# tgp-team/torch-geometric-pool

Hardware: AMD Instinct MI355X
Metric: pooled nodes/sec (Reduce+Connect) on batched graphs (higher is better)
Workload: dtype f32; 1 GPU; DiffPool dense S^T X / S^T A S, batch=32 graphs N=1024 K=128 F=64 (BASELINE configs[1]); graphs_per_gpu=32, nodes_per_graph=1024, clusters=128, features=64, parallelism=graph-sharded x1

## Files before the change

torch-geometric-pool_amd/csrc/dense.hip:

```cpp
#include <stdlib.h>

#include "common.h"
#include "gemm_mfma.h"
#include "dense_post.h"
#include "dense_graph_kernels.h"

namespace tgp {

static const int kStage2Tile = getenv("TGP_STAGE2_TILE") ? atoi(getenv("TGP_STAGE2_TILE")) : 0;
static const int kStage2TileM = getenv("TGP_STAGE2_TILE_M") ? atoi(getenv("TGP_STAGE2_TILE_M")) : 0;
struct DensePlan {
  int splits, tile, tile_m;
  int k_per_split;
  size_t u_floats, aslab_floats, xslab_floats, post_floats, colsum_floats;
};

static DensePlan dense_plan(int64_t B, int64_t N, int64_t K, int64_t F, bool with_gram = false) {
  DensePlan p;
  p.tile = (kStage2Tile == 64 || kStage2Tile == 128) ? kStage2Tile : 64;
  p.tile_m = (kStage2TileM == 64 || kStage2TileM == 128) ? kStage2TileM : p.tile;
  const int64_t T = p.tile, TM = p.tile_m;
  const int64_t tiles = ((K + TM - 1) / TM) * ((with_gram ? 2 : 1) * ((K + T - 1) / T) + ((F + T - 1) / T));
  const int64_t base = B * (tiles > 0 ? tiles : 1);
  const int64_t max_splits = (N + 4 * BK - 1) / (4 * BK);
  const int64_t cus = 256;
  int64_t splits = 1;
  double best = 1e30;
  for (int64_t sp = 1; sp <= 32 && sp <= (max_splits > 0 ? max_splits : 1); ++sp) {
    const int64_t wgs = base * sp;
    const int64_t ksteps = ((N + sp - 1) / sp + BK - 1) / BK;
    const int64_t per_cu = (wgs + cus - 1) / cus, resident = per_cu < 4 ? per_cu : 4;
    const double cost = static_cast<double>((per_cu + 3) / 4) * static_cast<double>(ksteps + 3) *
                        static_cast<double>(2 + resident) * (1.0 + 0.01 * sp);
    if (cost < best) { best = cost; splits = sp; }
  }
  static const int force_splits = getenv("TGP_STAGE2_SPLITS") ? atoi(getenv("TGP_STAGE2_SPLITS")) : 0;
  if (force_splits > 0 && force_splits <= max_splits) splits = force_splits;
  int64_t kps = (N + splits - 1) / splits;
  kps = (kps + BK - 1) / BK * BK;
  splits = (N + kps - 1) / kps;
  if (splits < 1) splits = 1;
  p.splits = static_cast<int>(splits);
  p.k_per_split = static_cast<int>(kps);
  p.u_floats = static_cast<size_t>(B) * N * K;
  const int64_t fold = fold_tiles(N, K, F) <= PR_MAX_SPLITS ? fold_tiles(N, K, F) : 0;
  const int64_t slabs = splits > fold ? splits : fold;
  const int64_t parts = splits * ((K + 63) / 64) > fold ? splits * ((K + 63) / 64) : fold;
  p.aslab_floats = static_cast<size_t>(B) * slabs * K * K;
  p.xslab_floats = static_cast<size_t>(B) * slabs * K * F;
  p.post_floats = post_ws_floats(B, K);
  p.colsum_floats = static_cast<size_t>(B) * parts * K;
  return p;
}

}

using namespace tgp;

extern "C" size_t tgp_dense_pool_workspace_bytes(int64_t B, int64_t N, int64_t K, int64_t F) {
  if (B <= 0 || N <= 0 || K <= 0) return 256;
  const DensePlan p = dense_plan(B, N, K, F > 0 ? F : 0);
  return align_up(p.u_floats * 4) + align_up(p.aslab_floats * 4) + align_up(p.xslab_floats * 4) +
         align_up(p.post_floats * 4) + align_up(p.colsum_floats * 4) + 256;
}

static bool dense_pool_small_ok(int64_t B, int64_t N, int64_t K, int64_t F) {
  static const int no_small = getenv("TGP_NO_SMALL_GRAPH_KERNEL") ? 1 : 0;
  return !no_small && N <= SG_N && K <= SG_K && F <= SG_K && B >= 64;
}

extern "C" int tgp_dense_pool_is_small(int64_t B, int64_t N, int64_t K, int64_t F) {
  return dense_pool_small_ok(B, N, K, F) ? 1 : 0;
}

static int dense_pool_impl(const float* S, const float* A, const float* X, int64_t B, int64_t N, int64_t K, int64_t F,
                           int flags, float eps, const int64_t* graph_sizes, float* x_pool, float* adj_raw,
                           float* adj_pool, float* mincut_terms, float loss_eps, void* ws, size_t ws_bytes,
                           void* stream_);
static int dense_pool_tiled(const float* S, const float* A, const float* X, int64_t B, int64_t N, int64_t K, int64_t F,
                            int flags, float eps, float* x_pool, float* adj_raw, float* adj_pool, float* U, int64_t ldu,
                            float* gram, const DensePlan& p, Carver& cv, hipStream_t stream, bool keep_u = true);

extern "C" int tgp_dense_pool_f32(const float* S, const float* A, const float* X, int64_t B, int64_t N,
                                  int64_t K, int64_t F, int flags, float eps, const int64_t* graph_sizes,
                                  float* x_pool,
                                  float* adj_raw, float* adj_pool, void* ws, size_t ws_bytes, void* stream_) {
  return dense_pool_impl(S, A, X, B, N, K, F, flags, eps, graph_sizes, x_pool, adj_raw, adj_pool, nullptr, 0.f, ws,
                         ws_bytes, stream_);
}

extern "C" int tgp_dense_pool_mincut_f32(const float* S, const float* A, const float* X, int64_t B, int64_t N,
                                         int64_t K, int64_t F, int flags, float eps, float loss_eps, float* x_pool,
                                         float* adj_raw, float* adj_pool, float* mincut_terms, void* ws,
                                         size_t ws_bytes, void* stream_) {
  TGP_REQUIRE(mincut_terms && A, TGP_ERR_INVALID, "tgp_dense_pool_mincut_f32: mincut_terms / A is null");
  TGP_REQUIRE(dense_pool_small_ok(B, N, K, F), TGP_ERR_INVALID,
              "tgp_dense_pool_mincut_f32: only batches the one-wave-per-graph kernel takes (tgp_dense_pool_is_small)");
  return dense_pool_impl(S, A, X, B, N, K, F, flags, eps, nullptr, x_pool, adj_raw, adj_pool, mincut_terms, loss_eps,
                         ws, ws_bytes, stream_);
}

extern "C" int tgp_dense_pool_select_f32(const float* X, const float* A, const float* W, const float* bias,
                                         const unsigned char* mask, int64_t B, int64_t N, int64_t K, int64_t F,
                                         int flags, float eps, float loss_eps, float* S_out, float* x_pool,
// ... 140 lines not shown
    (void)hipFuncSetAttribute(reinterpret_cast<const void*>(dense_pool_small_kernel<false, true>),
                              hipFuncAttributeMaxDynamicSharedMemorySize,
                              static_cast<int>(SG_WAVES * SG_WAVE_FLOATS * sizeof(float)));
    hipLaunchKernelGGL((dense_pool_small_kernel<false, true>), dim3(grid), dim3(64 * SG_WAVES),
                       SG_WAVES * SG_WAVE_FLOATS * sizeof(float), stream, q);
    return check_launch("tgp_dense_pool_f32(small)");
  }
  static const int no_medium = getenv("TGP_NO_MEDIUM_GRAPH_KERNEL") ? 1 : 0;
  static const int kMediumMinGraphs = getenv("TGP_MEDIUM_MIN_GRAPHS") ? atoi(getenv("TGP_MEDIUM_MIN_GRAPHS")) : 8;
  static const int kMediumMaxLds = getenv("TGP_MEDIUM_MAX_LDS") ? atoi(getenv("TGP_MEDIUM_MAX_LDS")) : 152 * 1024;
  if (!no_medium && K <= 64 && B >= kMediumMinGraphs && reinterpret_cast<uintptr_t>(S) % 4 == 0) {
    const int64_t npad = (N + 31) / 32 * 32;
    const size_t lds = K <= 32 ? medium_lds_bytes<1>(npad) : medium_lds_bytes<2>(npad);
    const bool fits32 = static_cast<int64_t>(N) * (N > F ? N : F) * 4 < (1ll << 31) - 4096;
    if (lds <= static_cast<size_t>(kMediumMaxLds) && fits32) {
      MediumArgs q{S, want_a ? A : nullptr, want_x ? X : nullptr, static_cast<int>(B), static_cast<int>(N),
                   static_cast<int>(K), static_cast<int>(F), flags, eps, want_x ? x_pool : nullptr,
                   want_a ? adj_raw : nullptr, want_a ? adj_pool : nullptr, static_cast<int>(npad), graph_sizes};
      static const int force_waves = getenv("TGP_MEDIUM_WAVES") ? atoi(getenv("TGP_MEDIUM_WAVES")) : 0;
      const int64_t strips = (want_a ? (N + 31) / 32 : 0) + (want_x ? (F + 31) / 32 : 0);
      const bool eight = force_waves ? force_waves == 8 : (strips >= 8 && lds > 80 * 1024);
      const dim3 g(static_cast<unsigned>(B));
      if (K <= 32) {
        if (eight) hipLaunchKernelGGL((dense_pool_medium_kernel<1, 4, 8>), g, dim3(512), lds, stream, q);
        else hipLaunchKernelGGL((dense_pool_medium_kernel<1>), g, dim3(256), lds, stream, q);
      } else {
        if (eight) hipLaunchKernelGGL((dense_pool_medium_kernel<2, 2, 8>), g, dim3(512), lds, stream, q);
        else hipLaunchKernelGGL((dense_pool_medium_kernel<2, 2>), g, dim3(256), lds, stream, q);
      }
      return check_launch("tgp_dense_pool_f32(medium)");
    }
  }
  TGP_REQUIRE(ws && ws_bytes >= tgp_dense_pool_workspace_bytes(B, N, K, F), TGP_ERR_WORKSPACE,
              "tgp_dense_pool_f32: workspace too small");
  const DensePlan p = dense_plan(B, N, K, F);
  Carver cv(ws);
  float* U = cv.take<float>(p.u_floats);
  return dense_pool_tiled(S, A, X, B, N, K, F, flags, eps, x_pool, adj_raw, adj_pool, U, K, nullptr, p, cv, stream,
                          false);
}

static int dense_pool_tiled(const float* S, const float* A, const float* X, int64_t B, int64_t N, int64_t K, int64_t F,
                            int flags, float eps, float* x_pool, float* adj_raw, float* adj_pool, float* U, int64_t ldu,
                            float* gram, const DensePlan& p, Carver& cv, hipStream_t stream, bool keep_u) {
  const bool want_x = X && x_pool && F > 0;
  const bool want_a = A && (adj_raw || adj_pool);
  float* aslab = cv.take<float>(p.aslab_floats);
  float* xslab = cv.take<float>(p.xslab_floats);
  float* postws = cv.take<float>(p.post_floats);
  float* colpart = cv.take<float>(p.colsum_floats);
  float* gslab = gram ? cv.take<float>(p.aslab_floats) : nullptr;

  const int fold = (want_a && !keep_u && !gram) ? fold_tiles(N, K, F) : 0;
  if (fold > 0 && fold <= PR_MAX_SPLITS && static_cast<size_t>(B) * fold * K * K <= p.aslab_floats &&
      post_rows_ok(K, flags, aslab, adj_raw, adj_pool) &&
      reinterpret_cast<uintptr_t>(xslab) % 16 == 0) {
    GemmArgs g{};
    g.A = A; g.lda = N; g.sA = N * N;
    g.M = static_cast<int>(N); g.Kd = static_cast<int>(N);
    g.rhs[0] = GemmRhs{S, aslab, static_cast<int>(K), K, K, N * K, static_cast<long>(fold) * K * K, K * K};
    if (want_x) g.rhs[1] = GemmRhs{X, xslab, static_cast<int>(F), F, F, N * F, static_cast<long>(fold) * K * F, K * F};
    g.splits = 1; g.k_per_split = static_cast<int>((N + BK - 1) / BK * BK);
    g.colsum = colpart;
    g.colsum_skip_diag = (flags & TGP_REMOVE_SELF_LOOPS) ? 1 : 0;
    const bool folded = (flags & TGP_ADJ_TRANSPOSED) ? launch_gemm_fold<true>(g, static_cast<int>(B), stream)
                                                     : launch_gemm_fold<false>(g, static_cast<int>(B), stream);
    if (folded) {
      PostRowsArgs r{};
      r.slab = aslab; r.splits = fold; r.s_split = K * K; r.s_batch = static_cast<long>(fold) * K * K;
      r.colsum = (flags & TGP_DEGREE_NORM) ? colpart : nullptr; r.tiles_m = 1;
      r.K = static_cast<int>(K); r.flags = flags; r.eps = eps; r.raw = adj_raw; r.dst = adj_pool;
      if (want_x) {
        r.xslab = xslab; r.xs_split = K * F; r.xs_batch = static_cast<long>(fold) * K * F;
        r.F = static_cast<int>(F); r.x_pool = x_pool;
      }
      const unsigned grid = static_cast<unsigned>(B * ((K + PR_ROWS - 1) / PR_ROWS));
      r.main_blocks = static_cast<int>(grid);
      hipLaunchKernelGGL(post_rows_kernel, dim3(grid), dim3(512), 0, stream, r);
      return check_launch("tgp_dense_pool_f32");
    }
  }
  if (want_a) {
    GemmArgs g{};
    g.A = A; g.lda = N; g.sA = N * N;
    g.M = static_cast<int>(N); g.Kd = static_cast<int>(N);
    g.rhs[0] = GemmRhs{S, U, static_cast<int>(K), K, ldu, N * K, N * ldu, 0};
    g.splits = 1; g.k_per_split = static_cast<int>((N + BK - 1) / BK * BK);
    if (flags & TGP_ADJ_TRANSPOSED) launch_gemm_skip_zeros<true>(g, static_cast<int>(B), stream);
    else launch_gemm_skip_zeros<false>(g, static_cast<int>(B), stream);
  }
  if (want_a || want_x) {
    GemmArgs h{};
    h.A = S; h.lda = K; h.sA = N * K;
    h.M = static_cast<int>(K); h.Kd = static_cast<int>(N);
    h.splits = p.splits; h.k_per_split = p.k_per_split;
    h.force_bm = p.tile_m; h.force_bn = p.tile;
    const GemmRhs ra{U, aslab, static_cast<int>(K), ldu, K, N * ldu, static_cast<long>(p.splits) * K * K, K * K};
    const GemmRhs rx{X, xslab, static_cast<int>(F), F, F, N * F, static_cast<long>(p.splits) * K * F, K * F};
    const GemmRhs rg{S, gslab, static_cast<int>(K), K, K, N * K, static_cast<long>(p.splits) * K * K, K * K};
    int nr = 0;
    if (want_a) h.rhs[nr++] = ra;
    if (want_x) h.rhs[nr++] = rx;
    if (gram) h.rhs[nr++] = rg;
    if (want_a && post_rows_ok(K, flags, aslab, adj_raw, adj_pool) && p.tile == 64 && p.tile_m == 64 &&
        p.splits <= PR_MAX_SPLITS && p.splits * ((K + 63) / 64) <= 2 * PR_MAX_SPLITS) {
      h.colsum = colpart;
      h.colsum_skip_diag = (flags & TGP_REMOVE_SELF_LOOPS) ? 1 : 0;
    }
    int tiles_m = 0;
    const bool have_colsum = launch_gemm<true>(h, static_cast<int>(B), stream, &tiles_m);
    if (have_colsum) {
      PostRowsArgs r{};
      r.slab = aslab; r.splits = p.splits; r.s_split = K * K; r.s_batch = static_cast<long>(p.splits) * K * K;
      r.colsum = (flags & TGP_DEGREE_NORM) ? colpart : nullptr; r.tiles_m = tiles_m;
      r.K = static_cast<int>(K); r.flags = flags; r.eps = eps; r.raw = adj_raw; r.dst = adj_pool;
      if (want_x) {
        r.xslab = xslab; r.xs_split = K * F; r.xs_batch = static_cast<long>(p.splits) * K * F;
        r.F = static_cast<int>(F); r.x_pool = x_pool;
      }
      unsigned grid = static_cast<unsigned>(B * ((K + PR_ROWS - 1) / PR_ROWS));
      r.main_blocks = static_cast<int>(grid);
      if (gram) {
        r.gslab = gslab; r.gram = gram;
        grid *= 2;
      }
      hipLaunchKernelGGL(post_rows_kernel, dim3(grid), dim3(512), 0, stream, r);
      return check_launch("tgp_dense_pool_f32");
    }
  }
  if (gram) {
    const long total = K * K;
    int gx = static_cast<int>((total + 255) / 256);
    if (gx > 64) gx = 64;
    hipLaunchKernelGGL(combine_slabs_kernel, dim3(gx, static_cast<unsigned>(B)), dim3(256), 0, stream, gslab,
                       p.splits, K * K, static_cast<long>(p.splits) * K * K, total, gram);
  }
  bool x_done = !want_x;
  if (want_a) {
    PostArgs q{};
    q.src = aslab; q.splits = p.splits; q.s_split = K * K; q.s_batch = static_cast<long>(p.splits) * K * K;
    q.ld_src = K; q.K = static_cast<int>(K); q.flags = flags; q.eps = eps; q.raw = adj_raw; q.dst = adj_pool;
    const XCombineArgs xc{xslab, p.splits, K * F, static_cast<long>(p.splits) * K * F, K * F, x_pool, 0};
    if (launch_post(q, B, postws, stream, want_x ? &xc : nullptr)) x_done = true;
  }
  if (!x_done) {
    const long total = K * F;
    int gx = static_cast<int>((total + 255) / 256);
    if (gx > 64) gx = 64;
    hipLaunchKernelGGL(combine_slabs_kernel, dim3(gx, static_cast<unsigned>(B)), dim3(256), 0, stream, xslab,
                       p.splits, K * F, static_cast<long>(p.splits) * K * F, total, x_pool);
  }
  return check_launch("tgp_dense_pool_f32");
}

extern "C" size_t tgp_dense_pool_train_workspace_bytes(int64_t B, int64_t N, int64_t K, int64_t F) {
  if (B <= 0 || N <= 0 || K <= 0) return 256;
  size_t best = 0;
  for (int with_gram = 0; with_gram < 2; ++with_gram) {
    const DensePlan p = dense_plan(B, N, K, F > 0 ? F : 0, with_gram != 0);
    const size_t bytes = 2 * align_up(p.aslab_floats * 4) + align_up(p.xslab_floats * 4) + align_up(p.post_floats * 4) +
                         align_up(p.colsum_floats * 4) + 256;
    if (bytes > best) best = bytes;
  }
  return best;
}

extern "C" int tgp_dense_pool_train_fwd_f32(const float* S, const float* A, const float* X, int64_t B, int64_t N,
                                            int64_t K, int64_t F, int flags, float eps, float* U, int64_t ldu,
                                            float* x_pool, float* adj_raw, float* adj_pool, float* gram, void* ws,
                                            size_t ws_bytes, void* stream_) {
  hipStream_t stream = static_cast<hipStream_t>(stream_);
  TGP_REQUIRE(B > 0 && N > 0 && K > 0 && F >= 0, TGP_ERR_INVALID, "tgp_dense_pool_train_fwd_f32: empty or negative size");
  TGP_REQUIRE(S && A && U && adj_raw && (F == 0 || (X && x_pool)), TGP_ERR_INVALID,
              "tgp_dense_pool_train_fwd_f32: null pointer");
  TGP_REQUIRE(ldu >= K, TGP_ERR_INVALID, "tgp_dense_pool_train_fwd_f32: ldu < K");
  TGP_REQUIRE(N < (1ll << 31) && K <= 16000 && F < (1ll << 31) && B < 65536 && N * ldu * 4 < (1ll << 31) - 4096,
              TGP_ERR_RANGE, "tgp_dense_pool_train_fwd_f32: dimension too large");
  TGP_REQUIRE(ws && ws_bytes >= tgp_dense_pool_train_workspace_bytes(B, N, K, F), TGP_ERR_WORKSPACE,
              "tgp_dense_pool_train_fwd_f32: workspace too small");
// ... 746 lines not shown
```

torch-geometric-pool_amd/csrc/dense_post.h:

```cpp
#pragma once
#include <stdlib.h>

#include "common.h"

namespace tgp {

constexpr int POST_BLOCKS = 64;

struct PostArgs {
  const float* src;
  int splits;
  long s_split, s_batch, ld_src;
  int K, flags;
  float eps;
  float* raw;
  float* dst;
  float* dvec;
  float* maxpart;
  int transpose_src;
};

template <int VEC>
__global__ __launch_bounds__(256) void post_combine_kernel(PostArgs p) {
  const int b = blockIdx.y, K = p.K;
// ... 344 lines not shown
      }
      __syncthreads();
    }
  }
  const bool by_cols = p.flags & TGP_SUM_AXIS_ROWS, ewn = p.flags & TGP_EDGE_WEIGHT_NORM;
  float mx = 0.f;
  for (int e = tid * 4; e < kk; e += 4096) {
    float4 t = *reinterpret_cast<const float4*>(m + e);
    if (p.flags & TGP_DEGREE_NORM) {
      const int i = e / K, j = e - i * K;
      const float di = dv[i];
      const float4 dj = *reinterpret_cast<const float4*>(dv + j);
      if (by_cols) {
        t.x = (t.x / dj.x) / di; t.y = (t.y / dj.y) / di; t.z = (t.z / dj.z) / di; t.w = (t.w / dj.w) / di;
      } else {
        t.x = (t.x / di) / dj.x; t.y = (t.y / di) / dj.y; t.z = (t.z / di) / dj.z; t.w = (t.w / di) / dj.w;
      }
    }
    if (ewn) {
      mx = nan_max(nan_max(mx, nan_max(fabsf(t.x), fabsf(t.y))), nan_max(fabsf(t.z), fabsf(t.w)));
      *reinterpret_cast<float4*>(m + e) = t;
    } else {
      *reinterpret_cast<float4*>(dstb + e) = t;
    }
  }
  if (!ewn) return;
#pragma unroll
  for (int d = 32; d > 0; d >>= 1) mx = nan_max(mx, __shfl_xor(mx, d, WAVE));
  if (lane == 0) s_max[w] = mx;
  __syncthreads();
  float gm = 0.f;
#pragma unroll
  for (int q = 0; q < 16; ++q) gm = nan_max(gm, s_max[q]);
  if (gm == 0.f) gm = 1.f;
  for (int e = tid * 4; e < kk; e += 4096) {
    float4 t = *reinterpret_cast<const float4*>(m + e);
    t.x = t.x / gm; t.y = t.y / gm; t.z = t.z / gm; t.w = t.w / gm;
    *reinterpret_cast<float4*>(dstb + e) = t;
  }
}

struct PostRowsArgs {
  const float* slab; int splits; long s_split, s_batch;
  const float* colsum; int tiles_m;
  int K, flags; float eps;
  float* raw; float* dst;
  const float* xslab; long xs_split, xs_batch; int F; float* x_pool;
  int main_blocks; const float* gslab; float* gram;
};

constexpr int PR_ROWS = 16;
constexpr int PR_MAX_SPLITS = 8;

__global__ __launch_bounds__(512) void post_rows_kernel(PostRowsArgs p) {
  __shared__ float s_d[1024];
  const int K = p.K, tid = threadIdx.x;
  const int blocks_per_graph = (K + PR_ROWS - 1) / PR_ROWS;
  if (p.gram && static_cast<int>(blockIdx.x) >= p.main_blocks) {
    const int id = blockIdx.x - p.main_blocks;
    const int gb_ = id / blocks_per_graph, grb = id - gb_ * blocks_per_graph;
    const int rows = K - grb * PR_ROWS < PR_ROWS ? K - grb * PR_ROWS : PR_ROWS;
    const long base = static_cast<long>(grb) * PR_ROWS * K;
    const float* src = p.gslab + static_cast<long>(gb_) * p.s_batch + base;
    float* dst = p.gram + static_cast<long>(gb_) * K * K + base;
    for (int e = tid * 4; e < rows * K; e += 2048) {
      float4 t = *reinterpret_cast<const float4*>(src + e);
      for (int sp = 1; sp < p.splits; ++sp) {
        const float4 v = *reinterpret_cast<const float4*>(src + sp * p.s_split + e);
        t.x = __fadd_rn(t.x, v.x); t.y = __fadd_rn(t.y, v.y); t.z = __fadd_rn(t.z, v.z); t.w = __fadd_rn(t.w, v.w);
      }
      *reinterpret_cast<float4*>(dst + e) = t;
    }
    return;
  }
  const int b = blockIdx.x / blocks_per_graph, rb = blockIdx.x - b * blocks_per_graph;
  const int i0 = rb * PR_ROWS;
  const float* sb = p.slab + static_cast<long>(b) * p.s_batch;
  const bool rsl = p.flags & TGP_REMOVE_SELF_LOOPS, dn = (p.flags & TGP_DEGREE_NORM) && p.colsum;
  const int kq = K >> 2;
  float4 acc[2];
  bool mine[2];
  int ei[2], ej[2];
#pragma unroll
  for (int u = 0; u < 2; ++u) {
    const int e = tid + u * 512;
    const int il = e / kq, jq = e - il * kq;
    ei[u] = i0 + il; ej[u] = jq * 4;
    mine[u] = il < PR_ROWS && ei[u] < K;
    float4 v[PR_MAX_SPLITS];
    const float* q = sb + (mine[u] ? static_cast<long>(ei[u]) * K + ej[u] : 0);
#pragma unroll
    for (int sp = 0; sp < PR_MAX_SPLITS; ++sp)
      v[sp] = *reinterpret_cast<const float4*>(q + (sp < p.splits ? sp * p.s_split : 0));
    float4 t = v[0];
#pragma unroll
    for (int sp = 1; sp < PR_MAX_SPLITS; ++sp)
      if (sp < p.splits) {
        t.x = __fadd_rn(t.x, v[sp].x); t.y = __fadd_rn(t.y, v[sp].y);
        t.z = __fadd_rn(t.z, v[sp].z); t.w = __fadd_rn(t.w, v[sp].w);
      }
    acc[u] = t;
  }
  const int xrows = K - i0 < PR_ROWS ? K - i0 : PR_ROWS;
  const int xcount = p.x_pool ? xrows * p.F : 0;
  const float* xb = p.x_pool ? p.xslab + static_cast<long>(b) * p.xs_batch + static_cast<long>(i0) * p.F : sb;
  float xv[2][PR_MAX_SPLITS];
#pragma unroll
  for (int u = 0; u < 2; ++u) {
// ... 148 lines not shown
```

torch-geometric-pool_amd/csrc/gemm_mfma.h:

```cpp
#pragma once
#include <stdlib.h>
#include <type_traits>

#include "common.h"

namespace tgp {


typedef float f32x16 __attribute__((ext_vector_type(16)));
typedef float f32x4 __attribute__((ext_vector_type(4)));

constexpr int BK = 32;
#ifndef TGP_OPERAND_PREFETCH
#define TGP_OPERAND_PREFETCH 1
#endif
#ifndef TGP_LOAD_AT
#define TGP_LOAD_AT 7
#endif
#ifndef TGP_STORE_AT
#define TGP_STORE_AT 3
#endif
#ifndef TGP_STEADY_LOOP
#define TGP_STEADY_LOOP 1
#endif
#ifndef TGP_SPREAD
#define TGP_SPREAD 1
#endif
#ifndef TGP_MIRROR_ROWS
#define TGP_MIRROR_ROWS 1
#endif
#ifndef TGP_VEC_EPILOGUE
#define TGP_VEC_EPILOGUE 1
#endif

constexpr int LDA_ROWMAJOR = BK + 1;

#ifndef TGP_SPARSE_CHUNK_GROUPS
#define TGP_SPARSE_CHUNK_GROUPS 224
#endif
#ifndef TGP_SPARSE_WIDE_GROUPS
#define TGP_SPARSE_WIDE_GROUPS 896
#endif
#ifndef TGP_DENSE_RUN
#define TGP_DENSE_RUN 2
#endif
#ifndef TGP_FOLD_SKIP_ACC
#define TGP_FOLD_SKIP_ACC 1
#endif
#ifndef TGP_FOLD_SPLIT
#define TGP_FOLD_SPLIT 1
#endif

struct GemmRhs {
  const float* Bm;
  float* C;
  int Nc;
  long ldb, ldc, sB, sC, sCsplit;
};

struct GemmArgs {
  const float* A;
  long lda, sA;
  int M, Kd;
  GemmRhs rhs[3];
  int tiles_m, tiles_n0, tiles_n;
  int tiles_n1;
  int splits;
  int k_per_split;
  const int64_t* k_ptr;
  const int64_t* m_ptr;
  const float* resid;
  long ldr, sR;
  float* partial;
  int force_bm, force_bn;
  const int64_t* sizes;
  int accumulate;
  float* colsum;
  int colsum_skip_diag;
  int symmetric;
};

__device__ __forceinline__ int tile_row(int t) {
  const int g = t >> 3, r = t & 7;
  return 4 * (g & 7) + (r & 3) + 32 * (r >> 2) + 64 * (g >> 3);
}

#ifdef TGP_GEMM_STAMPS
__device__ unsigned long long* g_gemm_stamps = nullptr;
__device__ int g_gemm_reverse = 0;
#define TGP_STAMP(slot)                                                                        \
  do {                                                                                          \
    if (g_gemm_stamps && threadIdx.x == 0)                                                      \
      g_gemm_stamps[static_cast<long>(blockIdx.x) * 16 + (slot)] = __builtin_amdgcn_s_memrealtime(); \
  } while (0)
#else
#define TGP_STAMP(slot) do {} while (0)
#endif

__device__ __forceinline__ float4 ld4_guarded(const float* p, bool ok) {
  return ok ? *reinterpret_cast<const float4*>(p) : make_float4(0.f, 0.f, 0.f, 0.f);
}

template <bool A_KMAJOR, bool ALIGNED, int BM, int BN, int MODE, int WN = 2>
// ... 684 lines not shown
#pragma unroll
      for (int i = 0; i < 2; ++i) a_at[i] = lq * BN + ((wm * 32 + 16 * i + l15) ^ (lq << 4));
#pragma unroll
      for (int j = 0; j < 2; ++j) u_at[j] = lq * 192 + ((wn * 32 + 16 * j + l15) ^ (lq << 4));
      const int x_at = lq * 192 + ((BN + wn * 16 + l15) ^ (lq << 4));
      float a[2][2], b[2][2];
      auto fetch_u = [&](int s) {
#pragma unroll
        for (int i = 0; i < 2; ++i) a[s & 1][i] = Sf[4 * s * BN + a_at[i]];
#pragma unroll
        for (int j = 0; j < 2; ++j) b[s & 1][j] = UXf[4 * s * 192 + u_at[j]];
      };
      auto fetch_x = [&](int s) {
#pragma unroll
        for (int i = 0; i < 2; ++i) a[s & 1][i] = Sf[4 * s * BN + a_at[i]];
        b[s & 1][0] = UXf[4 * s * 192 + x_at];
      };
      fetch_u(0);
#pragma unroll
      for (int s = 0; s < 32; ++s) {
        if (s + 1 < 32) fetch_u(s + 1);
        else fetch_x(0);
#pragma unroll
        for (int j = 0; j < 2; ++j)
#pragma unroll
          for (int i = 0; i < 2; ++i)
            d[i][j] = __builtin_amdgcn_mfma_f32_16x16x4f32(a[s & 1][i], b[s & 1][j], d[i][j], 0, 0, 0);
        if (s + 1 < 32) __builtin_amdgcn_sched_group_barrier(0x100, 4, 0);
        else __builtin_amdgcn_sched_group_barrier(0x100, 3, 0);
        __builtin_amdgcn_sched_group_barrier(0x008, 4, 0);
        __builtin_amdgcn_sched_barrier(0);
      }
      TGP_STAMP(9);
      float cpart[2][2];
      if (g.colsum) {
#pragma unroll
        for (int i = 0; i < 2; ++i)
#pragma unroll
          for (int j = 0; j < 2; ++j) {
            const int col = wn * 32 + 16 * j + l15;
            float cs = 0.f;
#pragma unroll
            for (int q = 0; q < 4; ++q) {
              if (q) cs = __shfl_up(cs, 16, 64);
#pragma unroll
              for (int r = 0; r < 4; ++r) {
                const int row = wm * 32 + 16 * i + 4 * lq + r;
                cs = __fadd_rn(cs, (row >= Nc || (g.colsum_skip_diag && row == col)) ? 0.f : d[i][j][r]);
              }
            }
            cpart[i][j] = cs;
          }
      }
      float* Ca = R.C + static_cast<long>(batch) * R.sC + static_cast<long>(tm) * R.sCsplit;
      float* cp = Ca + static_cast<long>(tid >> 5) * R.ldc + (tid & 31) * 4;
      const long cp_step = 32 * R.ldc;
      float4 pv = make_float4(0.f, 0.f, 0.f, 0.f);
#pragma unroll
      for (int s = 0; s < 32; ++s) {
        if (s == G_FREE) __syncthreads();
        if (s == G_FREE + G_PARK) {
          __syncthreads();
          TGP_STAMP(10);
        }
        if (s + 1 < 32) fetch_x(s + 1);
#pragma unroll
        for (int i = 0; i < 2; ++i) d[i][2] = __builtin_amdgcn_mfma_f32_16x16x4f32(a[s & 1][i], b[s & 1][0], d[i][2], 0, 0, 0);
        if (s + 1 < 32) __builtin_amdgcn_sched_group_barrier(0x100, 3, 0);
        __builtin_amdgcn_sched_group_barrier(0x008, 2, 0);
        if (s >= G_FREE && s < G_FREE + G_PARK) {
#pragma unroll
          for (int h = 0; h < PARK_PER; ++h) {
            const int e = PARK_PER * (s - G_FREE) + h, i = e >> 3, j = (e >> 2) & 1, r = e & 3;
            const int p = wm * 32 + 16 * i + 4 * lq + r;
            UXf[p * 192 + ((wn * 32 + 16 * j + l15) ^ ((lq & 1) << 4))] = d[i][j][r];
          }
        }
        if (s >= G_FREE + G_PARK && s < G_FREE + G_PARK + 8) {
          const int e = s - (G_FREE + G_PARK), q = e >> 1;
          const int row = (tid >> 5) + 32 * q, c4 = (tid & 31) * 4;
          if ((e & 1) == 0) pv = *reinterpret_cast<const float4*>(UXf + row * 192 + (c4 ^ (((row >> 2) & 1) << 4)));
          else if (row < Nc && c4 < Nc) *reinterpret_cast<float4*>(cp + q * cp_step) = pv;
        }
        __builtin_amdgcn_sched_barrier(0);
      }
      TGP_STAMP(11);
      if (F) {
        float* Cx = RX.C + static_cast<long>(batch) * RX.sC + static_cast<long>(tm) * RX.sCsplit;
        const int col = wn * 16 + l15;
#pragma unroll
        for (int i = 0; i < 2; ++i)
#pragma unroll
          for (int r = 0; r < 4; ++r) {
            const int row = wm * 32 + 16 * i + 4 * lq + r;
            if (row < Nc && col < F) Cx[static_cast<long>(row) * RX.ldc + col] = d[i][2][r];
          }
      }
      if (g.colsum) {
        __syncthreads();
        float* part = smem;
        if (lq == 3) {
#pragma unroll
          for (int i = 0; i < 2; ++i)
#pragma unroll
            for (int j = 0; j < 2; ++j) part[(2 * wm + i) * BN + wn * 32 + 16 * j + l15] = cpart[i][j];
        }
        __syncthreads();
        if (tid < Nc) {
          float tot = 0.f;
#pragma unroll
          for (int qq = 0; qq < 8; ++qq) tot = __fadd_rn(tot, part[qq * BN + tid]);
          g.colsum[(static_cast<long>(batch) * g.tiles_m + tm) * Nc + tid] = tot;
        }
      }
      TGP_STAMP(3);
      return;
    }
    {
      int a_at[2], b_at[3];
#pragma unroll
      for (int i = 0; i < 2; ++i) a_at[i] = lq * BN + ((wm * 32 + 16 * i + l15) ^ (lq << 4));
#pragma unroll
      for (int j = 0; j < 3; ++j) b_at[j] = lq * 192 + ((wn * 48 + 16 * j + l15) ^ (lq << 4));
      float a[2][2], b[2][3];
      auto fetch = [&](int s) {
#pragma unroll
        for (int i = 0; i < 2; ++i) a[s & 1][i] = Sf[4 * s * BN + a_at[i]];
#pragma unroll
        for (int j = 0; j < 3; ++j) b[s & 1][j] = UXf[4 * s * 192 + b_at[j]];
      };
      fetch(0);
#pragma unroll
      for (int s = 0; s < 32; ++s) {
        if (s + 1 < 32) fetch(s + 1);
#pragma unroll
        for (int j = 0; j < 3; ++j)
#pragma unroll
          for (int i = 0; i < 2; ++i)
            d[i][j] = __builtin_amdgcn_mfma_f32_16x16x4f32(a[s & 1][i], b[s & 1][j], d[i][j], 0, 0, 0);
        if (s + 1 < 32) __builtin_amdgcn_sched_group_barrier(0x100, 5, 0);
        __builtin_amdgcn_sched_group_barrier(0x008, 6, 0);
        __builtin_amdgcn_sched_barrier(0);
      }
    }
    TGP_STAMP(9);
    __syncthreads();
    bool used[3];
#pragma unroll
    for (int j = 0; j < 3; ++j) {
// ... 213 lines not shown
static bool launch_gemm(GemmArgs g, int batches, hipStream_t stream, int* tiles_m_out = nullptr) {
  int64_t max_nc = g.rhs[1].Bm && g.rhs[1].Nc > g.rhs[0].Nc ? g.rhs[1].Nc : g.rhs[0].Nc;
  const bool third = g.rhs[1].Bm && g.rhs[2].Bm;
  if (third && g.rhs[2].Nc > max_nc) max_nc = g.rhs[2].Nc;
  const TileCfg t = pick_tile(g.M, max_nc, static_cast<int64_t>(batches) * g.splits, g);
  g.tiles_m = cdiv(g.M, t.bm);
  g.tiles_n0 = cdiv(g.rhs[0].Nc, t.bn);
  g.tiles_n = g.tiles_n0 + (g.rhs[1].Bm ? cdiv(g.rhs[1].Nc, t.bn) : 0);
  g.tiles_n1 = 0;
  if (third) {
    g.tiles_n1 = g.tiles_n;
    g.tiles_n += cdiv(g.rhs[2].Nc, t.bn);
  }
  if (tiles_m_out) *tiles_m_out = g.tiles_m;
  if (t.bm == 64 && t.bn == 64 && g.colsum) {
    launch_gemm_cfg<A_KMAJOR, 64, 64, 2>(g, batches, stream);
    return true;
  }
  if (t.bm == 64 && t.bn == 64) launch_gemm_cfg<A_KMAJOR, 64, 64>(g, batches, stream);
  else if (t.bm == 64) launch_gemm_cfg<A_KMAJOR, 64, 128>(g, batches, stream);
  else if (t.bn == 64) launch_gemm_cfg<A_KMAJOR, 128, 64>(g, batches, stream);
  else launch_gemm_cfg<A_KMAJOR, 128, 128, 0, 4>(g, batches, stream);
  return false;
}

template <bool A_KMAJOR>
static void launch_gemm_skip_zeros(GemmArgs g, int batches, hipStream_t stream) {
  if (g.splits != 1 || g.accumulate || g.rhs[1].Bm || g.colsum || g.m_ptr || g.k_ptr || !gemm_aligned(g, A_KMAJOR)) {
    launch_gemm<A_KMAJOR>(g, batches, stream);
    return;
  }
  constexpr int BM = 128, BN = 128, WN = 4;
  const int tiles_m = cdiv(g.M, BM), tiles_n = cdiv(g.rhs[0].Nc, BN);
  const int nwg = batches * tiles_m * tiles_n;
  if (nwg < 256) {
    launch_gemm<A_KMAJOR>(g, batches, stream);
    return;
  }
  g.tiles_m = tiles_m;
  g.tiles_n0 = g.tiles_n = tiles_n;
  g.tiles_n1 = 0;
  constexpr size_t lds = A_KMAJOR ? 2 * (BM * LDA_ROWMAJOR + BK * BN) * sizeof(float) + 2 * 16 * sizeof(unsigned)
                                  : 2 * 128 * BN * sizeof(float) + (2 * 16 + 16 * 256) * sizeof(unsigned);
  static_assert(A_KMAJOR || 2 * 128 * BN >= 2 * (BM * LDA_ROWMAJOR + BK * BN) + 2 * 16, "MODE 3: the wide chunks cover the stages");
  if constexpr (!A_KMAJOR)
    (void)hipFuncSetAttribute(reinterpret_cast<const void*>(gemm_f32_mfma_kernel<A_KMAJOR, true, BM, BN, 3, WN>),
                              hipFuncAttributeMaxDynamicSharedMemorySize, static_cast<int>(lds));
  hipLaunchKernelGGL((gemm_f32_mfma_kernel<A_KMAJOR, true, BM, BN, 3, WN>), dim3(nwg), dim3(BM * 2 * WN), lds, stream, g);
}

constexpr int FOLD_BM = 128, FOLD_MAX_F = 64;
static int fold_tiles(int64_t N, int64_t K, int64_t F) {
  return (K <= 128 && K % 4 == 0 && F <= FOLD_MAX_F && F % 4 == 0) ? cdiv(N, FOLD_BM) : 0;
}
template <bool A_KMAJOR>
static bool launch_gemm_fold(GemmArgs g, int batches, hipStream_t stream) {
  constexpr int BM = FOLD_BM, BN = 128, WN = 4;
  const GemmRhs x = g.rhs[1];
  g.rhs[1] = GemmRhs{};
  const long lim = (1l << 31) - 4096;
  if (!gemm_aligned(g, A_KMAJOR) || g.rhs[0].Nc > BN ||
      (x.Bm && (reinterpret_cast<uintptr_t>(x.Bm) % 4 != 0 || x.Nc > FOLD_MAX_F || (static_cast<long>(g.Kd) + BM) * x.ldb * 4 >= lim)))
    return false;
  g.rhs[1] = x;
  g.tiles_m = cdiv(g.M, BM);
  g.tiles_n0 = g.tiles_n = 1;
  g.tiles_n1 = 0;
  g.splits = 1;
  const int nwg = batches * g.tiles_m;
  if (nwg < 256) return false;
  constexpr size_t lds = (BM * BN + BM * 192) * sizeof(float);
  static_assert(BM * BN + BM * 192 >= BM * 196 + 8 * BN && BM * 196 + 8 * BN >= 2 * (BM * LDA_ROWMAJOR + BK * BN) + 2 * 16,
                "MODE 4: the tail's operands cover its result tile, which covers the k-loop's stages");
  static_assert(BM * BN + BM * 192 >= 2 * 128 * BN + 2 * 16 + 16 * 256, "MODE 4: ... and the wide front-end's two Bm chunks, records and turn areas");
  (void)hipFuncSetAttribute(reinterpret_cast<const void*>(gemm_f32_mfma_kernel<A_KMAJOR, true, BM, BN, 4, WN>),
                            hipFuncAttributeMaxDynamicSharedMemorySize, static_cast<int>(lds));
  hipLaunchKernelGGL((gemm_f32_mfma_kernel<A_KMAJOR, true, BM, BN, 4, WN>), dim3(nwg), dim3(BM * 2 * WN), lds, stream, g);
  return true;
}

static int launch_gemm_residual(GemmArgs g, int batches, hipStream_t stream, bool dry_run = false) {
  TileCfg t = pick_tile(g.M, g.rhs[0].Nc, batches, g);
  if (g.symmetric && g.Kd <= 8 * BK && !g.force_bm && !g.force_bn && t.bm == 128 && t.bn == 128) t = TileCfg{64, 64};
  g.tiles_m = cdiv(g.M, t.bm);
  g.tiles_n0 = g.tiles_n = cdiv(g.rhs[0].Nc, t.bn);
  if (dry_run) return g.tiles_m * g.tiles_n;
  static const int no_sym = getenv("TGP_LINK_LOSS_FULL") ? atoi(getenv("TGP_LINK_LOSS_FULL")) : 0;
  if (t.bm != t.bn || g.M != g.rhs[0].Nc || g.rhs[0].Bm != g.A || g.rhs[0].sB != g.sA || g.rhs[0].ldb != g.lda || no_sym)
    g.symmetric = 0;
  if (t.bm == 64 && t.bn == 64) launch_gemm_cfg<false, 64, 64, 1>(g, batches, stream);
  else if (t.bm == 64) launch_gemm_cfg<false, 64, 128, 1>(g, batches, stream);
  else if (t.bn == 64) launch_gemm_cfg<false, 128, 64, 1>(g, batches, stream);
  else launch_gemm_cfg<false, 128, 128, 1, 4>(g, batches, stream);
  return g.tiles_m * g.tiles_n;
}

}
```

Baseline: 563.9 million nodes/s.

## Store fold GEMM partials as MFMA-native 16x16 blocks, skip LDS transpose

The fold GEMM now writes its per-tile S^T A S and S^T X partial slabs straight from the MFMA accumulators as 16x16 fragment blocks, using buffer stores with a write-through hint. Previously the accumulators were parked in LDS, synchronised and re-read to build row-major stores. A new templated post_rows_kernel variant reads this blocked layout, sums the splits and writes the row-major pooled outputs. This drops the LDS staging and the two barriers from the GEMM epilogue, but the blocked layout makes the post-processing addressing more complex and may pad the slabs.

```diff
diff --git a/torch-geometric-pool_amd/csrc/dense.hip b/torch-geometric-pool_amd/csrc/dense.hip
--- a/torch-geometric-pool_amd/csrc/dense.hip
+++ b/torch-geometric-pool_amd/csrc/dense.hip
@@ -50,6 +50,10 @@
   p.xslab_floats = static_cast<size_t>(B) * slabs * K * F;
   p.post_floats = post_ws_floats(B, K);
   p.colsum_floats = static_cast<size_t>(B) * parts * K;
+  const size_t fold_a = static_cast<size_t>(B * fold * fold_slab_floats(K, K));
+  const size_t fold_x = static_cast<size_t>(B * fold * fold_slab_floats(K, F));
+  if (fold_a > p.aslab_floats) p.aslab_floats = fold_a;
+  if (fold_x > p.xslab_floats) p.xslab_floats = fold_x;
   return p;
 }
 
@@ -296,14 +300,16 @@
   float* gslab = gram ? cv.take<float>(p.aslab_floats) : nullptr;
 
   const int fold = (want_a && !keep_u && !gram) ? fold_tiles(N, K, F) : 0;
-  if (fold > 0 && fold <= PR_MAX_SPLITS && static_cast<size_t>(B) * fold * K * K <= p.aslab_floats &&
+  const long a_slab = fold_slab_floats(K, K), x_slab = fold_slab_floats(K, F);
+  if (fold > 0 && fold <= PR_MAX_SPLITS && static_cast<size_t>(B) * fold * a_slab <= p.aslab_floats &&
+      static_cast<size_t>(B) * fold * x_slab <= p.xslab_floats &&
       post_rows_ok(K, flags, aslab, adj_raw, adj_pool) &&
       reinterpret_cast<uintptr_t>(xslab) % 16 == 0) {
     GemmArgs g{};
     g.A = A; g.lda = N; g.sA = N * N;
     g.M = static_cast<int>(N); g.Kd = static_cast<int>(N);
-    g.rhs[0] = GemmRhs{S, aslab, static_cast<int>(K), K, K, N * K, static_cast<long>(fold) * K * K, K * K};
-    if (want_x) g.rhs[1] = GemmRhs{X, xslab, static_cast<int>(F), F, F, N * F, static_cast<long>(fold) * K * F, K * F};
+    g.rhs[0] = GemmRhs{S, aslab, static_cast<int>(K), K, K, N * K, fold * a_slab, a_slab};
+    if (want_x) g.rhs[1] = GemmRhs{X, xslab, static_cast<int>(F), F, F, N * F, fold * x_slab, x_slab};
     g.splits = 1; g.k_per_split = static_cast<int>((N + BK - 1) / BK * BK);
     g.colsum = colpart;
     g.colsum_skip_diag = (flags & TGP_REMOVE_SELF_LOOPS) ? 1 : 0;
@@ -311,16 +317,16 @@
                                                      : launch_gemm_fold<false>(g, static_cast<int>(B), stream);
     if (folded) {
       PostRowsArgs r{};
-      r.slab = aslab; r.splits = fold; r.s_split = K * K; r.s_batch = static_cast<long>(fold) * K * K;
+      r.slab = aslab; r.splits = fold; r.s_split = a_slab; r.s_batch = fold * a_slab;
       r.colsum = (flags & TGP_DEGREE_NORM) ? colpart : nullptr; r.tiles_m = 1;
       r.K = static_cast<int>(K); r.flags = flags; r.eps = eps; r.raw = adj_raw; r.dst = adj_pool;
       if (want_x) {
-        r.xslab = xslab; r.xs_split = K * F; r.xs_batch = static_cast<long>(fold) * K * F;
+        r.xslab = xslab; r.xs_split = x_slab; r.xs_batch = fold * x_slab;
         r.F = static_cast<int>(F); r.x_pool = x_pool;
       }
       const unsigned grid = static_cast<unsigned>(B * ((K + PR_ROWS - 1) / PR_ROWS));
       r.main_blocks = static_cast<int>(grid);
-      hipLaunchKernelGGL(post_rows_kernel, dim3(grid), dim3(512), 0, stream, r);
+      hipLaunchKernelGGL(post_rows_kernel<TGP_FOLD_BLOCKS != 0>, dim3(grid), dim3(512), 0, stream, r);
       return check_launch("tgp_dense_pool_f32");
     }
   }
@@ -368,7 +374,7 @@
         r.gslab = gslab; r.gram = gram;
         grid *= 2;
       }
-      hipLaunchKernelGGL(post_rows_kernel, dim3(grid), dim3(512), 0, stream, r);
+      hipLaunchKernelGGL(post_rows_kernel<false>, dim3(grid), dim3(512), 0, stream, r);
       return check_launch("tgp_dense_pool_f32");
     }
   }
diff --git a/torch-geometric-pool_amd/csrc/dense_post.h b/torch-geometric-pool_amd/csrc/dense_post.h
--- a/torch-geometric-pool_amd/csrc/dense_post.h
+++ b/torch-geometric-pool_amd/csrc/dense_post.h
@@ -420,8 +420,83 @@
 constexpr int PR_ROWS = 16;
 constexpr int PR_MAX_SPLITS = 8;
 
+template <bool BLOCKS>
 __global__ __launch_bounds__(512) void post_rows_kernel(PostRowsArgs p) {
   __shared__ float s_d[1024];
+  if constexpr (BLOCKS) {
+    const int K = p.K, tid = threadIdx.x, kb = (K + 15) >> 4;
+    const int b = blockIdx.x / kb, rb = blockIdx.x - b * kb, i0 = rb * PR_ROWS;
+    const bool rsl = p.flags & TGP_REMOVE_SELF_LOOPS, dn = (p.flags & TGP_DEGREE_NORM) && p.colsum;
+    const int bc = tid >> 6, lq = (tid >> 4) & 3;
+    const int c = 16 * bc + (tid & 15), r0 = i0 + 4 * lq;
+    const float* sb = p.slab + static_cast<long>(b) * p.s_batch;
+    const bool mine = bc < kb && c < K && r0 < K;
+    float4 t;
+    {
+      float4 v[PR_MAX_SPLITS];
+      const float* q = sb + (mine ? static_cast<long>(rb) * kb * 256 + 4 * tid : 0);
+#pragma unroll
+      for (int sp = 0; sp < PR_MAX_SPLITS; ++sp)
+        v[sp] = *reinterpret_cast<const float4*>(q + (sp < p.splits ? sp * p.s_split : 0));
+      t = v[0];
+#pragma unroll
+      for (int sp = 1; sp < PR_MAX_SPLITS; ++sp)
+        if (sp < p.splits) {
+          t.x = __fadd_rn(t.x, v[sp].x); t.y = __fadd_rn(t.y, v[sp].y);
+          t.z = __fadd_rn(t.z, v[sp].z); t.w = __fadd_rn(t.w, v[sp].w);
+        }
+    }
+    const int F = p.x_pool ? p.F : 0, fb = (F + 15) >> 4;
+    const bool xmine = bc < fb && c < F && r0 < K;
+    float4 xv[PR_MAX_SPLITS];
+    {
+      const float* xq = xmine ? p.xslab + static_cast<long>(b) * p.xs_batch + static_cast<long>(rb) * fb * 256 + 4 * tid : sb;
+#pragma unroll
+      for (int sp = 0; sp < PR_MAX_SPLITS; ++sp)
+        xv[sp] = *reinterpret_cast<const float4*>(xq + ((xmine && sp < p.splits) ? sp * p.xs_split : 0));
+    }
+    if (dn) {
+      for (int j = tid; j < K; j += 512) {
+        const float* cs = p.colsum + static_cast<long>(b) * p.splits * K + j;
+        float pv[PR_MAX_SPLITS];
+#pragma unroll
+        for (int qq = 0; qq < PR_MAX_SPLITS; ++qq) pv[qq] = cs[qq < p.splits ? static_cast<long>(qq) * K : 0];
+        float cc = 0.f;
+#pragma unroll
+        for (int qq = 0; qq < PR_MAX_SPLITS; ++qq)
+          if (qq < p.splits) cc = __fadd_rn(cc, pv[qq]);
+        s_d[j] = sqrtf(clamp_min(cc, p.eps));
+      }
+    }
+    float* rawb = p.raw ? p.raw + static_cast<long>(b) * K * K : nullptr;
+    float* dstb = p.dst ? p.dst + static_cast<long>(b) * K * K : nullptr;
+    __syncthreads();
+    if (mine) {
+      float tv[4] = {t.x, t.y, t.z, t.w};
+      const float dj = dn ? s_d[c] : 1.f;
+#pragma unroll
+      for (int r = 0; r < 4; ++r) {
+        const long off = static_cast<long>(r0 + r) * K + c;
+        if (rawb) rawb[off] = tv[r];
+        if (!dstb) continue;
+        if (rsl && r0 + r == c) tv[r] = 0.f;
+        if (dn) tv[r] = (tv[r] / dj) / s_d[r0 + r];
+        dstb[off] = tv[r];
+      }
+    }
+    if (xmine) {
+      float4 v = xv[0];
+#pragma unroll
+      for (int sp = 1; sp < PR_MAX_SPLITS; ++sp)
+        if (sp < p.splits) {
+          v.x = __fadd_rn(v.x, xv[sp].x); v.y = __fadd_rn(v.y, xv[sp].y);
+          v.z = __fadd_rn(v.z, xv[sp].z); v.w = __fadd_rn(v.w, xv[sp].w);
+        }
+      float* xo = p.x_pool + static_cast<long>(b) * K * F + static_cast<long>(r0) * F + c;
+      xo[0] = v.x; xo[F] = v.y; xo[2 * F] = v.z; xo[3 * F] = v.w;
+    }
+    return;
+  }
   const int K = p.K, tid = threadIdx.x;
   const int blocks_per_graph = (K + PR_ROWS - 1) / PR_ROWS;
   if (p.gram && static_cast<int>(blockIdx.x) >= p.main_blocks) {
diff --git a/torch-geometric-pool_amd/csrc/gemm_mfma.h b/torch-geometric-pool_amd/csrc/gemm_mfma.h
--- a/torch-geometric-pool_amd/csrc/gemm_mfma.h
+++ b/torch-geometric-pool_amd/csrc/gemm_mfma.h
@@ -49,6 +49,16 @@
 #endif
 #ifndef TGP_FOLD_SPLIT
 #define TGP_FOLD_SPLIT 1
+#endif
+#ifndef TGP_FOLD_BLOCKS
+#define TGP_FOLD_BLOCKS 1
+#endif
+#ifndef TGP_FOLD_SLAB_WT
+#define TGP_FOLD_SLAB_WT 1
+#endif
+#if !TGP_FOLD_SPLIT
+#undef TGP_FOLD_BLOCKS
+#define TGP_FOLD_BLOCKS 0
 #endif
 
 struct GemmRhs {
@@ -839,49 +849,89 @@
             cpart[i][j] = cs;
           }
       }
-      float* Ca = R.C + static_cast<long>(batch) * R.sC + static_cast<long>(tm) * R.sCsplit;
-      float* cp = Ca + static_cast<long>(tid >> 5) * R.ldc + (tid & 31) * 4;
-      const long cp_step = 32 * R.ldc;
-      float4 pv = make_float4(0.f, 0.f, 0.f, 0.f);
-#pragma unroll
-      for (int s = 0; s < 32; ++s) {
-        if (s == G_FREE) __syncthreads();
-        if (s == G_FREE + G_PARK) {
-          __syncthreads();
-          TGP_STAMP(10);
-        }
-        if (s + 1 < 32) fetch_x(s + 1);
-#pragma unroll
-        for (int i = 0; i < 2; ++i) d[i][2] = __builtin_amdgcn_mfma_f32_16x16x4f32(a[s & 1][i], b[s & 1][0], d[i][2], 0, 0, 0);
-        if (s + 1 < 32) __builtin_amdgcn_sched_group_barrier(0x100, 3, 0);
-        __builtin_amdgcn_sched_group_barrier(0x008, 2, 0);
-        if (s >= G_FREE && s < G_FREE + G_PARK) {
-#pragma unroll
-          for (int h = 0; h < PARK_PER; ++h) {
-            const int e = PARK_PER * (s - G_FREE) + h, i = e >> 3, j = (e >> 2) & 1, r = e & 3;
-            const int p = wm * 32 + 16 * i + 4 * lq + r;
-            UXf[p * 192 + ((wn * 32 + 16 * j + l15) ^ ((lq & 1) << 4))] = d[i][j][r];
+      if constexpr (TGP_FOLD_BLOCKS) {
+        typedef unsigned int u32x4 __attribute__((ext_vector_type(4)));
+        constexpr int WT = TGP_FOLD_SLAB_WT ? 16 : 0;
+        const int kb = (Nc + 15) >> 4, fb = (F + 15) >> 4;
+        float* Ca = R.C + static_cast<long>(batch) * R.sC + static_cast<long>(tm) * R.sCsplit;
+        const __amdgpu_buffer_rsrc_t rsrc_c = __builtin_amdgcn_make_buffer_rsrc(Ca, 0, kb * kb * 1024, 0x00020000);
+        int voff_c[2][2];
+#pragma unroll
+        for (int i = 0; i < 2; ++i)
+#pragma unroll
+          for (int j = 0; j < 2; ++j) {
+            const int br = 2 * wm + i, bc = 2 * wn + j;
+            voff_c[i][j] = (br < kb && bc < kb) ? (br * kb + bc) * 1024 + lane * 16 : OOB;
           }
-        }
-        if (s >= G_FREE + G_PARK && s < G_FREE + G_PARK + 8) {
-          const int e = s - (G_FREE + G_PARK), q = e >> 1;
-          const int row = (tid >> 5) + 32 * q, c4 = (tid & 31) * 4;
-          if ((e & 1) == 0) pv = *reinterpret_cast<const float4*>(UXf + row * 192 + (c4 ^ (((row >> 2) & 1) << 4)));
-          else if (row < Nc && c4 < Nc) *reinterpret_cast<float4*>(cp + q * cp_step) = pv;
-        }
-        __builtin_amdgcn_sched_barrier(0);
-      }
-      TGP_STAMP(11);
-      if (F) {
-        float* Cx = RX.C + static_cast<long>(batch) * RX.sC + static_cast<long>(tm) * RX.sCsplit;
-        const int col = wn * 16 + l15;
-#pragma unroll
-        for (int i = 0; i < 2; ++i)
-#pragma unroll
-          for (int r = 0; r < 4; ++r) {
-            const int row = wm * 32 + 16 * i + 4 * lq + r;
-            if (row < Nc && col < F) Cx[static_cast<long>(row) * RX.ldc + col] = d[i][2][r];
+#pragma unroll
+        for (int s = 0; s < 32; ++s) {
+          if (s == 12) TGP_STAMP(10);
+          if (s + 1 < 32) fetch_x(s + 1);
+#pragma unroll
+          for (int i = 0; i < 2; ++i) d[i][2] = __builtin_amdgcn_mfma_f32_16x16x4f32(a[s & 1][i], b[s & 1][0], d[i][2], 0, 0, 0);
+          if (s + 1 < 32) __builtin_amdgcn_sched_group_barrier(0x100, 3, 0);
+          __builtin_amdgcn_sched_group_barrier(0x008, 2, 0);
+          if (s < 4)
+            __builtin_amdgcn_raw_buffer_store_b128(__builtin_bit_cast(u32x4, d[s >> 1][s & 1]), rsrc_c,
+                                                   voff_c[s >> 1][s & 1], 0, WT);
+          __builtin_amdgcn_sched_barrier(0);
+        }
+        TGP_STAMP(11);
+        if (F) {
+          float* Cx = RX.C + static_cast<long>(batch) * RX.sC + static_cast<long>(tm) * RX.sCsplit;
+          const __amdgpu_buffer_rsrc_t rsrc_cx = __builtin_amdgcn_make_buffer_rsrc(Cx, 0, kb * fb * 1024, 0x00020000);
+#pragma unroll
+          for (int i = 0; i < 2; ++i) {
+            const int br = 2 * wm + i;
+            __builtin_amdgcn_raw_buffer_store_b128(__builtin_bit_cast(u32x4, d[i][2]), rsrc_cx,
+                                                   (br < kb && wn < fb) ? (br * fb + wn) * 1024 + lane * 16 : OOB, 0, WT);
           }
+        }
+      } else {
+        float* Ca = R.C + static_cast<long>(batch) * R.sC + static_cast<long>(tm) * R.sCsplit;
+        float* cp = Ca + static_cast<long>(tid >> 5) * R.ldc + (tid & 31) * 4;
+        const long cp_step = 32 * R.ldc;
+        float4 pv = make_float4(0.f, 0.f, 0.f, 0.f);
+#pragma unroll
+        for (int s = 0; s < 32; ++s) {
+          if (s == G_FREE) __syncthreads();
+          if (s == G_FREE + G_PARK) {
+            __syncthreads();
+            TGP_STAMP(10);
+          }
+          if (s + 1 < 32) fetch_x(s + 1);
+#pragma unroll
+          for (int i = 0; i < 2; ++i) d[i][2] = __builtin_amdgcn_mfma_f32_16x16x4f32(a[s & 1][i], b[s & 1][0], d[i][2], 0, 0, 0);
+          if (s + 1 < 32) __builtin_amdgcn_sched_group_barrier(0x100, 3, 0);
+          __builtin_amdgcn_sched_group_barrier(0x008, 2, 0);
+          if (s >= G_FREE && s < G_FREE + G_PARK) {
+#pragma unroll
+            for (int h = 0; h < PARK_PER; ++h) {
+              const int e = PARK_PER * (s - G_FREE) + h, i = e >> 3, j = (e >> 2) & 1, r = e & 3;
+              const int p = wm * 32 + 16 * i + 4 * lq + r;
+              UXf[p * 192 + ((wn * 32 + 16 * j + l15) ^ ((lq & 1) << 4))] = d[i][j][r];
+            }
+          }
+          if (s >= G_FREE + G_PARK && s < G_FREE + G_PARK + 8) {
+            const int e = s - (G_FREE + G_PARK), q = e >> 1;
+            const int row = (tid >> 5) + 32 * q, c4 = (tid & 31) * 4;
+            if ((e & 1) == 0) pv = *reinterpret_cast<const float4*>(UXf + row * 192 + (c4 ^ (((row >> 2) & 1) << 4)));
+            else if (row < Nc && c4 < Nc) *reinterpret_cast<float4*>(cp + q * cp_step) = pv;
+          }
+          __builtin_amdgcn_sched_barrier(0);
+        }
+        TGP_STAMP(11);
+        if (F) {
+          float* Cx = RX.C + static_cast<long>(batch) * RX.sC + static_cast<long>(tm) * RX.sCsplit;
+          const int col = wn * 16 + l15;
+#pragma unroll
+          for (int i = 0; i < 2; ++i)
+#pragma unroll
+            for (int r = 0; r < 4; ++r) {
+              const int row = wm * 32 + 16 * i + 4 * lq + r;
+              if (row < Nc && col < F) Cx[static_cast<long>(row) * RX.ldc + col] = d[i][2][r];
+            }
+        }
       }
       if (g.colsum) {
         __syncthreads();
@@ -1201,6 +1251,9 @@
 constexpr int FOLD_BM = 128, FOLD_MAX_F = 64;
 static int fold_tiles(int64_t N, int64_t K, int64_t F) {
   return (K <= 128 && K % 4 == 0 && F <= FOLD_MAX_F && F % 4 == 0) ? cdiv(N, FOLD_BM) : 0;
+}
+static int64_t fold_slab_floats(int64_t rows, int64_t cols) {
+  return TGP_FOLD_BLOCKS ? ((rows + 15) / 16) * ((cols + 15) / 16) * 256 : rows * cols;
 }
 template <bool A_KMAJOR>
 static bool launch_gemm_fold(GemmArgs g, int batches, hipStream_t stream) {
```

New measurement: 601.2 million nodes/s, median of 6. 1.07x the previous value.
